# lucadellalib/ts-asr

Hardware: AMD Instinct MI355X
Metric: utterance-frames/sec (conformer-t_scratch training step, T=1000, B=32/GPU) (higher is better)
Workload: dtype bf16; 1 GPU; BASELINE.json configs[1]: conformer-t_scratch 12L d256 (+6L speaker encoder), mel [32,1000,80] + enrollment mel [32,500,80] + tokens [32,120], injection cat, dropout 0.1, lens 1.0; global_batch=32, grad_accumulation_factor=1, parallelism=dp1, hip_graph=True

## Files before the change

### include/tsasr_hip.h

```cpp
#ifndef TSASR_HIP_H
#define TSASR_HIP_H
#include <stddef.h>
#include <stdint.h>

#ifdef __cplusplus
extern "C" {
#endif

#define TSASR_F32 0
#define TSASR_BF16 1

#define TSASR_E_INVALID (-1)
#define TSASR_E_LAUNCH (-2)
#define TSASR_E_WORKSPACE (-3)

const char *tsasr_last_error(void);
int tsasr_version(void);
int tsasr_device_ok(void);

int tsasr_joint_fwd(const void *enc, const void *dec, const float *W, const float *bias, float *logits,
                    int B, int T, int U1, int J, int V, int ldl, int io_dtype, float slope, void *stream);

int tsasr_joint_f32_fwd(const float *enc, const float *dec, const float *W, const float *bias, float *logits, int B, int T, int U1, int J, int V,
                        int ldl, float slope, void *stream);
// ... 82 lines not shown
int tsasr_frontend_out_len(int n);
int tsasr_frontend_c1_fwd(const void *x, const float *w1, const float *b1, const float *w2, const float *b2, void *y1, void *y2,
                          int B, int T, int F, int C, int causal, int io_dtype, void *stream);
size_t tsasr_frontend_c1_bwd_workspace_bytes(int C);
int tsasr_frontend_c1_bwd(const void *x, const void *dy1, const void *dy2, float *dparams, int B, int T, int F, int C, int causal,
                          int io_dtype, void *workspace, size_t workspace_bytes, void *stream);
int tsasr_frontend_im2col(const void *x, void *A, int B, int T, int F, int C, int causal, int io_dtype, void *stream);
int tsasr_frontend_col2im(const void *dA, const void *dR, void *dx, int B, int T, int F, int C, int causal, int io_dtype, void *stream);

int tsasr_frontend_block_supported(int Fo, int C);
int tsasr_frontend_block_fwd(const void *x, const void *y1, const void *y2, const float *w1, const float *b1, const float *w2,
                             const float *b2, const float *g1, const float *be1, const float *g2, const float *be2, void *out,
                             float *stats, int B, int T, int F, int C, int causal, float slope, float eps, float p_inner,
                             unsigned long long seed_inner, float p_outer, unsigned long long seed_outer,
                             const unsigned long long *seed_dev, int io_dtype, void *stream);
size_t tsasr_frontend_block_dparams(int Fo, int C, int with_conv);
size_t tsasr_frontend_block_bwd_workspace_bytes(int Fo, int C, int with_conv);
int tsasr_frontend_block_bwd(const void *x, const void *y1, const void *y2, const void *dout, const float *w1, const float *b1,
                             const float *w2, const float *b2, const float *g1, const float *be1, const float *g2,
                             const float *stats, void *dy1, void *dy2, float *dparams, int B, int T, int F, int C, int causal,
                             float slope, float p_inner, unsigned long long seed_inner, float p_outer,
                             unsigned long long seed_outer, const unsigned long long *seed_dev, int io_dtype, void *workspace,
                             size_t workspace_bytes, void *stream);


size_t tsasr_relpos_attn_lds_bytes(void);
int tsasr_relpos_attn_fwd(const void *qkv, const void *pk, const float *bias_u, const float *bias_v, const int32_t *key_lens,
                          void *out, float *lse, int B, int T, int H, int Dh, float scale, int causal, float pdrop,
                          unsigned long long seed, const unsigned long long *seed_dev, int io_dtype, void *stream);
size_t tsasr_relpos_attn_fwd_workspace_bytes(int B, int T, int H);
int tsasr_relpos_attn_fwd_ws(const void *qkv, const void *pk, const float *bias_u, const float *bias_v, const int32_t *key_lens,
                             void *out, float *lse, int B, int T, int H, int Dh, float scale, int causal, float pdrop,
                             unsigned long long seed, const unsigned long long *seed_dev, int io_dtype, void *workspace,
                             size_t workspace_bytes, void *stream);
size_t tsasr_relpos_attn_bwd_workspace_bytes(int B, int T, int H);
int tsasr_relpos_attn_bwd(const void *qkv, const void *pk, const float *bias_u, const float *bias_v, const int32_t *key_lens,
                          const void *out, const void *dout, const float *lse, void *dqkv, void *dpk, float *d_bias_u,
                          float *d_bias_v, int B, int T, int H, int Dh, float scale, int causal, float pdrop,
                          unsigned long long seed, const unsigned long long *seed_dev, int io_dtype, void *workspace, size_t workspace_bytes,
                          void *stream);
int tsasr_relpos_dpk_defer(int on);
int tsasr_relpos_dpk_pending(void);
size_t tsasr_relpos_dpk_table_bytes(int max_jobs);
int tsasr_relpos_dpk_flush(void *table_host, void *table_dev, size_t table_bytes, void *stream);
void tsasr_relpos_dpk_discard(void);
size_t tsasr_relpos_attn_keepbits_bytes(int B, int T, int H);
void tsasr_relpos_attn_keepbits(void *bits);

int tsasr_accumulate_many(const void *table, int count, void *stream);
size_t tsasr_clip_adamw_workspace_bytes(void);
int tsasr_clip_adamw_step(float *p, void *p_bf16, const float *g, float *m, float *v, const float *hyper, float *norm_out, float *skipped_out,
                          long long n, float beta1, float beta2, float eps, float weight_decay, float max_norm, void *workspace,
                          size_t workspace_bytes, void *stream);

void tsasr_gemm_set_ring(int on);
void tsasr_gemm_set_lab_floor(int floor_mode);
void tsasr_gemm_set_plan(int tile, int splits);
size_t tsasr_gemm_bf16_workspace_bytes(int M, int N, int K, int out_dtype);
int tsasr_gemm_bf16(const void *A, const void *B, void *C, int M, int N, int K, long long lda, long long ldb, long long ldc,
                    int transA, int transB, int out_dtype, int accumulate, void *workspace, size_t workspace_bytes, void *stream);
int tsasr_gemm_f32(const float *A, const float *B, float *C, int M, int N, int K, long long lda, long long ldb, long long ldc, int transA,
                   int transB, int accumulate, void *stream);
int tsasr_gemm_bf16_nt_batched(const void *A, const void *const *btab, void *C, int M, int N, int K, long long lda, long long ldb,
                               long long ldc, long long c_batch, int nbatch, void *stream);
size_t tsasr_gemm_bf16_fused_workspace_bytes(int M, int N);
int tsasr_gemm_bf16_fused_mask_ok(int M, int N, int K);
int tsasr_gemm_bf16_fused(const void *A, const void *B, void *C, int M, int N, int K, long long lda, long long ldb, long long ldc,
                          int transA, int transB, int epi_mode, const float *bias, const void *y, long long ldy, float slope, float p,
                          unsigned long long seed, const unsigned long long *seed_dev, float *dbias, void *mask, void *workspace,
                          size_t workspace_bytes, void *stream);

int tsasr_lstm_cell_fwd(float *gates, float *c, void *h, int B, int U, int H, int t, int io_dtype, void *stream);
int tsasr_lstm_step_fwd(float *gates, float *c, void *h, const void *whh, int B, int U, int H, int t, int io_dtype, void *stream);
int tsasr_lstm_step_bwd(const float *gates, const float *c, const void *dout, void *dgates, const void *whhT, float *dc_io, int B, int U,
                        int H, int t, int io_dtype, void *stream);
int tsasr_lstm_cell_bwd(const float *gates, const float *c, const void *dout, const float *dh_rec, float *dc_io, void *dgates, int B,
                        int U, int H, int t, int io_dtype, void *stream);

size_t tsasr_fbank_workspace_bytes(int B, int T, int n_mels);
int tsasr_fbank_fwd(const float *wav, const float *window, const float *melmat, void *out, int B, int L, int T, int n_mels, int hop,
                    float top_db, float amin, int out_dtype, void *workspace, size_t workspace_bytes, void *stream);
int tsasr_sentence_norm_fwd(const void *x, const int32_t *lens, void *y, int B, int T, int F, float eps, int in_dtype, int out_dtype,
                            void *stream);

size_t tsasr_fbank_frames_workspace_bytes(int n_mels);
int tsasr_fbank_frames(const float *seg, const float *window, const float *melmat, float *out_db, int B, int Lseg, int F, int n_mels, int hop,
                       float amin, void *workspace, size_t workspace_bytes, void *stream);
size_t tsasr_running_norm_state_bytes(int B, int n_mels);
int tsasr_running_norm_fwd(const float *db, const int32_t *n_valid, void *state, void *y, int B, int F, int n_mels, float top_db, double eps,
                           int out_dtype, void *stream);

int tsasr_add_layernorm_fwd(const void *x, const float *bias, const void *res, void *s, void *y, float *mean, float *rstd,
                            const float *gamma, const float *beta, long long M, int D, float alpha, float p, unsigned long long seed,
                            const unsigned long long *seed_dev, const int32_t *valid_lens, int Trows, float eps, int io_dtype,
                            void *stream);
size_t tsasr_add_layernorm_bwd_workspace_bytes(long long M, int D);
int tsasr_add_layernorm_bwd(const void *dy, const void *dout, const void *s, const float *gamma, const float *mean, const float *rstd,
                            void *dres, void *dx, float *dgamma, float *dbeta, float *dbias, long long M, int D, float alpha, float p,
                            unsigned long long seed, const unsigned long long *seed_dev, const int32_t *valid_lens, int Trows,
                            int io_dtype, void *workspace, size_t workspace_bytes, void *stream);
int tsasr_linear_add_layernorm_ok(long long M, int N, int K, long long lda, long long ldw);
int tsasr_linear_add_layernorm_fwd(const void *A, long long lda, const void *W, long long ldw, const float *bias, const void *res, void *s,
                                   void *y, float *mean, float *rstd, const float *gamma, const float *beta, long long M, int N, int K,
                                   float alpha, float p, unsigned long long seed, const unsigned long long *seed_dev,
                                   const int32_t *valid_lens, int Trows, float eps, void *stream);
int tsasr_add_layernorm2_fwd(const void *x, const float *bias, const void *res, void *s, void *y, void *z, float *mean, float *rstd,
// ... 158 lines not shown
```

### ts-asr_amd/_capi.py

```python
import ctypes
import os

_HERE = os.path.dirname(os.path.abspath(__file__))
LIB_PATH = os.environ.get("TSASR_HIP_LIB") or os.path.join(_HERE, "lib", "libtsasr_hip.so")

F32, BF16 = 0, 1


class TsasrHipMissing(RuntimeError):
    pass


class TsasrHipError(RuntimeError):
    pass


_lib = None

c_void_p, c_int, c_float, c_size_t = ctypes.c_void_p, ctypes.c_int, ctypes.c_float, ctypes.c_size_t
c_double = ctypes.c_double
c_ll, c_ull = ctypes.c_longlong, ctypes.c_ulonglong

_PROTOS = {
    "tsasr_last_error": (ctypes.c_char_p, []),
# ... 16 lines not shown
    "tsasr_rnnt_align_workspace_bytes": (c_size_t, [c_int] * 3),
    "tsasr_rnnt_align": (c_int, [c_void_p, c_void_p, c_int, c_void_p, c_void_p, c_void_p, c_int, c_void_p] + [c_int] * 6 + [c_void_p, c_size_t, c_void_p]),
    "tsasr_layernorm_fwd": (c_int, [c_void_p] * 6 + [c_ll, c_int, c_float, c_float, c_int, c_void_p]),
    "tsasr_layernorm_bwd_workspace_bytes": (c_size_t, [c_ll, c_int]),
    "tsasr_layernorm_bwd": (c_int, [c_void_p] * 9 + [c_ll, c_int, c_float, c_int, c_void_p, c_size_t, c_void_p]),
    "tsasr_layernorm_bwd_add": (c_int, [c_void_p] * 10 + [c_ll, c_int, c_float, c_int, c_void_p, c_size_t, c_void_p]),
    "tsasr_seed_advance": (c_int, [c_void_p, c_ull, c_void_p]),
    "tsasr_bias_act_dropout_fwd": (c_int, [c_void_p] * 3 + [c_ll, c_int, c_float, c_float, c_ull, c_void_p, c_int, c_void_p]),
    "tsasr_colpart_workspace_bytes": (c_size_t, [c_ll, c_int]),
    "tsasr_bias_act_dropout_bwd": (c_int, [c_void_p] * 4 + [c_ll, c_int, c_float, c_float, c_ull, c_void_p, c_int, c_void_p, c_size_t, c_void_p]),
    "tsasr_dropout_add_fwd": (c_int, [c_void_p] * 4 + [c_ll, c_int, c_float, c_float, c_ull, c_void_p, c_void_p, c_int, c_int, c_void_p]),
    "tsasr_dropout_add_bwd": (c_int, [c_void_p] * 3 + [c_ll, c_int, c_float, c_float, c_ull, c_void_p, c_void_p, c_int, c_int, c_void_p, c_size_t, c_void_p]),
    "tsasr_dropout_add2_fwd": (c_int, [c_void_p] * 4 + [c_ll, c_int, c_float, c_float, c_ull, c_float, c_ull, c_void_p, c_void_p, c_int, c_int, c_void_p]),
    "tsasr_dropout_add2_bwd": (c_int, [c_void_p] * 4 + [c_ll, c_int, c_float, c_float, c_ull, c_float, c_ull, c_void_p, c_void_p, c_int, c_int, c_void_p, c_size_t, c_void_p]),
    "tsasr_colsum_workspace_bytes": (c_size_t, [c_ll, c_int]),
    "tsasr_colsum": (c_int, [c_void_p, c_void_p, c_ll, c_int, c_int, c_int, c_void_p, c_size_t, c_void_p]),
    "tsasr_convmod_fwd": (c_int, [c_void_p] * 10 + [c_int] * 5 + [c_float, c_float, c_int, c_void_p]),
    "tsasr_convmod_bwd_workspace_bytes": (c_size_t, [c_int] * 4),
    "tsasr_convmod_bwd": (c_int, [c_void_p] * 11 + [c_int] * 5 + [c_float, c_int, c_void_p, c_size_t, c_void_p]),
    "tsasr_frontend_out_len": (c_int, [c_int]),
    "tsasr_frontend_c1_fwd": (c_int, [c_void_p] * 7 + [c_int] * 6 + [c_void_p]),
    "tsasr_frontend_c1_bwd_workspace_bytes": (c_size_t, [c_int]),
    "tsasr_frontend_c1_bwd": (c_int, [c_void_p] * 4 + [c_int] * 6 + [c_void_p, c_size_t, c_void_p]),
    "tsasr_conv3x3s2_fwd": (c_int, [c_void_p] * 7 + [c_int] * 6 + [c_void_p]),
    "tsasr_conv3x3s2_wgrad_workspace_bytes": (c_size_t, [c_int] * 4),
    "tsasr_conv3x3s2_wgrad": (c_int, [c_void_p] * 5 + [c_int] * 6 + [c_void_p, c_size_t, c_void_p]),
    "tsasr_conv3x3s2_wgrad_filters": (c_int, [c_void_p] * 5 + [c_int] * 6 + [c_void_p, c_size_t, c_void_p]),
    "tsasr_conv3x3s2_dgrad_plan_bytes": (c_size_t, [c_int] * 4),
    "tsasr_conv3x3s2_dgrad_plan": (c_int, [c_int] * 4 + [c_void_p, c_size_t]),
    "tsasr_conv3x3s2_dgrad": (c_int, [c_void_p] * 5 + [c_int] * 6 + [c_void_p, c_size_t, c_void_p]),
    "tsasr_frontend_im2col": (c_int, [c_void_p] * 2 + [c_int] * 6 + [c_void_p]),
    "tsasr_frontend_col2im": (c_int, [c_void_p] * 3 + [c_int] * 6 + [c_void_p]),
    "tsasr_frontend_block_supported": (c_int, [c_int, c_int]),
    "tsasr_frontend_block_fwd": (c_int, [c_void_p] * 13 + [c_int] * 5 + [c_float, c_float, c_float, c_ull, c_float, c_ull, c_void_p, c_int, c_void_p]),
    "tsasr_frontend_block_dparams": (c_size_t, [c_int] * 3),
    "tsasr_frontend_block_bwd_workspace_bytes": (c_size_t, [c_int] * 3),
    "tsasr_frontend_block_bwd": (c_int, [c_void_p] * 15 + [c_int] * 5 + [c_float, c_float, c_ull, c_float, c_ull, c_void_p, c_int, c_void_p, c_size_t, c_void_p]),
    "tsasr_relpos_attn_lds_bytes": (c_size_t, []),
    "tsasr_relpos_attn_fwd": (c_int, [c_void_p] * 7 + [c_int] * 4 + [c_float, c_int, c_float, c_ull, c_void_p, c_int, c_void_p]),
    "tsasr_relpos_attn_fwd_workspace_bytes": (c_size_t, [c_int] * 3),
    "tsasr_relpos_attn_fwd_ws": (c_int, [c_void_p] * 7 + [c_int] * 4 + [c_float, c_int, c_float, c_ull, c_void_p, c_int, c_void_p, c_size_t, c_void_p]),
    "tsasr_relpos_attn_bwd_workspace_bytes": (c_size_t, [c_int] * 3),
    "tsasr_relpos_attn_bwd": (c_int, [c_void_p] * 12 + [c_int] * 4 + [c_float, c_int, c_float, c_ull, c_void_p, c_int, c_void_p, c_size_t, c_void_p]),
    "tsasr_relpos_dpk_defer": (c_int, [c_int]),
    "tsasr_relpos_dpk_pending": (c_int, []),
    "tsasr_relpos_dpk_table_bytes": (c_size_t, [c_int]),
    "tsasr_relpos_dpk_flush": (c_int, [c_void_p, c_void_p, c_size_t, c_void_p]),
    "tsasr_relpos_dpk_discard": (None, []),
    "tsasr_relpos_attn_keepbits_bytes": (c_size_t, [c_int] * 3),
    "tsasr_relpos_attn_keepbits": (None, [c_void_p]),
    "tsasr_accumulate_many": (c_int, [c_void_p, c_int, c_void_p]),
    "tsasr_clip_adamw_workspace_bytes": (c_size_t, []),
    "tsasr_clip_adamw_step": (c_int, [c_void_p] * 8 + [c_ll] + [c_float] * 5 + [c_void_p, c_size_t, c_void_p]),
    "tsasr_gemm_set_plan": (None, [c_int, c_int]),
    "tsasr_gemm_set_ring": (None, [c_int]),
    "tsasr_gemm_set_lab_floor": (None, [c_int]),
    "tsasr_gemm_bf16_workspace_bytes": (c_size_t, [c_int] * 4),
    "tsasr_gemm_f32": (c_int, [c_void_p] * 3 + [c_int] * 3 + [c_ll] * 3 + [c_int] * 3 + [c_void_p]),
    "tsasr_gemm_bf16_nt_batched": (c_int, [c_void_p] * 3 + [c_int] * 3 + [c_ll] * 4 + [c_int, c_void_p]),
    "tsasr_gemm_bf16_fused_workspace_bytes": (c_size_t, [c_int] * 2),
    "tsasr_gemm_bf16_fused": (c_int, [c_void_p] * 3 + [c_int] * 3 + [c_ll] * 3 + [c_int] * 3 + [c_void_p, c_void_p, c_ll, c_float, c_float, c_ull, c_void_p, c_void_p, c_void_p, c_void_p, c_size_t, c_void_p]),
    "tsasr_gemm_bf16_fused_mask_ok": (c_int, [c_int] * 3),
    "tsasr_gemm_bf16": (c_int, [c_void_p] * 3 + [c_int] * 3 + [c_ll] * 3 + [c_int] * 4 + [c_void_p, c_size_t, c_void_p]),
    "tsasr_lstm_step_fwd": (c_int, [c_void_p] * 4 + [c_int] * 5 + [c_void_p]),
    "tsasr_lstm_step_bwd": (c_int, [c_void_p] * 6 + [c_int] * 5 + [c_void_p]),
    "tsasr_lstm_cell_fwd": (c_int, [c_void_p] * 3 + [c_int] * 5 + [c_void_p]),
    "tsasr_lstm_cell_bwd": (c_int, [c_void_p] * 6 + [c_int] * 5 + [c_void_p]),
    "tsasr_fbank_workspace_bytes": (c_size_t, [c_int] * 3),
    "tsasr_fbank_fwd": (c_int, [c_void_p] * 4 + [c_int] * 5 + [c_float, c_float, c_int, c_void_p, c_size_t, c_void_p]),
    "tsasr_sentence_norm_fwd": (c_int, [c_void_p] * 3 + [c_int] * 3 + [c_float, c_int, c_int, c_void_p]),
    "tsasr_fbank_frames_workspace_bytes": (c_size_t, [c_int]),
    "tsasr_fbank_frames": (c_int, [c_void_p] * 4 + [c_int] * 5 + [c_float, c_void_p, c_size_t, c_void_p]),
    "tsasr_running_norm_state_bytes": (c_size_t, [c_int] * 2),
    "tsasr_running_norm_fwd": (c_int, [c_void_p] * 4 + [c_int] * 3 + [c_float, c_double, c_int, c_void_p]),
    "tsasr_add_layernorm_fwd": (c_int, [c_void_p] * 9 + [c_ll, c_int, c_float, c_float, c_ull, c_void_p, c_void_p, c_int, c_float, c_int, c_void_p]),
    "tsasr_add_layernorm_bwd_workspace_bytes": (c_size_t, [c_ll, c_int]),
    "tsasr_add_layernorm_bwd": (c_int, [c_void_p] * 11 + [c_ll, c_int, c_float, c_float, c_ull, c_void_p, c_void_p, c_int, c_int, c_void_p, c_size_t, c_void_p]),
    "tsasr_add_layernorm2_fwd": (c_int, [c_void_p] * 14 + [c_ll, c_int, c_float, c_float, c_ull, c_void_p, c_void_p, c_int, c_float, c_float, c_int, c_void_p]),
    "tsasr_add_layernorm2_bwd_workspace_bytes": (c_size_t, [c_ll, c_int]),
    "tsasr_add_layernorm2_bwd": (c_int, [c_void_p] * 18 + [c_ll, c_int, c_float, c_float, c_ull, c_void_p, c_void_p, c_int, c_int, c_void_p, c_size_t, c_void_p]),
    "tsasr_lstm_onehot_gates": (c_int, [c_void_p] * 6 + [c_int] * 6 + [c_void_p]),
    "tsasr_lstm_seq_persistent": (c_int, [c_int, c_int, c_int]),
    "tsasr_lstm_seq_workspace_bytes": (c_size_t, [c_int, c_int, c_int]),
    "tsasr_lstm_seq_fwd": (c_int, [c_void_p] * 4 + [c_int] * 4 + [c_void_p, c_size_t, c_void_p]),
    "tsasr_lstm_seq_bwd": (c_int, [c_void_p] * 5 + [c_int] * 4 + [c_void_p, c_size_t, c_void_p]),
    "tsasr_transpose_many_bf16": (c_int, [c_void_p, c_void_p, c_void_p, c_int, c_int, c_void_p]),
    "tsasr_reduce_defer": (c_int, [c_int]),
    "tsasr_reduce_pending": (c_int, []),
    "tsasr_reduce_discard": (None, []),
    "tsasr_reduce_table_bytes": (c_size_t, [c_int]),
    "tsasr_reduce_flush": (c_int, [c_void_p, c_void_p, c_size_t, c_void_p]),
    "tsasr_reduce_flush_stream": (c_int, [c_void_p, c_void_p, c_size_t, c_void_p]),
    "tsasr_mean_pool_fwd": (c_int, [c_void_p] * 3 + [c_int] * 4 + [c_void_p]),
    "tsasr_mean_pool_bwd": (c_int, [c_void_p] * 3 + [c_int] * 4 + [c_void_p]),
    "tsasr_abs_lengths": (c_int, [c_void_p] * 4 + [c_int, c_int, c_void_p]),
    "tsasr_inject_fwd": (c_int, [c_void_p] * 3 + [c_int] * 5 + [c_void_p]),
    "tsasr_inject_bwd": (c_int, [c_void_p] * 5 + [c_int] * 5 + [c_void_p]),
    "tsasr_greedy_decode": (c_int, [c_void_p] * 12 + [c_int] * 7 + [c_float, c_int, c_int, c_void_p]),
    "tsasr_greedy_decode_stream": (c_int, [c_void_p] * 14 + [c_int] * 7 + [c_float, c_int, c_int, c_void_p]),
    "tsasr_beam_search_workspace_bytes": (c_size_t, [c_int] * 6),
    "tsasr_beam_search": (c_int, [c_void_p] * 11 + [c_size_t] + [c_void_p] * 4 + [c_int] * 11 + [c_double, c_double, c_float, c_int, c_int, c_void_p]),
    "tsasr_beam_search_stream": (c_int, [c_void_p] * 11 + [c_size_t] + [c_void_p] * 5 + [c_int] * 12 + [c_double, c_double, c_float, c_int, c_int, c_void_p]),
    "tsasr_beam_search_timed_workspace_bytes": (c_size_t, [c_int] * 6),
    "tsasr_beam_search_timed": (c_int, [c_void_p] * 11 + [c_size_t] + [c_void_p] * 4 + [c_int] * 11 + [c_double, c_double, c_float, c_int, c_int, c_void_p, c_void_p]),
    "tsasr_beam_search_stream_timed": (c_int, [c_void_p] * 11 + [c_size_t] + [c_void_p] * 5 + [c_int] * 12 + [c_double, c_double, c_float, c_int, c_int, c_void_p, c_void_p]),
    "tsasr_beam_search_lm_workspace_bytes": (c_size_t, [c_int] * 9),
# ... 117 lines not shown
```

### ts-asr_amd/csrc/optim.hip

```cpp
#include <float.h>

#include "common.h"

#define OPT_PARTS 1024

__global__ __launch_bounds__(256) void sumsq_partials_kernel(const float *__restrict__ g, float *__restrict__ part, long long n) {
    __shared__ float red[4];
    const long long per = (((n + OPT_PARTS - 1) / OPT_PARTS) + 3) & ~3ll;
    const long long lo = min(n, (long long)blockIdx.x * per), hi = min(n, lo + per);
    const long long hi4 = lo + ((hi - lo) & ~3ll);
    float s0 = 0.f, s1 = 0.f, s2 = 0.f, s3 = 0.f;
    long long i = lo + threadIdx.x * 4;
    for (; i + 3 * 1024 + 4 <= hi4; i += 4 * 1024) {
        const float4 a = *reinterpret_cast<const float4 *>(g + i), b = *reinterpret_cast<const float4 *>(g + i + 1024);
        const float4 c = *reinterpret_cast<const float4 *>(g + i + 2048), d = *reinterpret_cast<const float4 *>(g + i + 3072);
        s0 += a.x * a.x + a.y * a.y + a.z * a.z + a.w * a.w;
        s1 += b.x * b.x + b.y * b.y + b.z * b.z + b.w * b.w;
        s2 += c.x * c.x + c.y * c.y + c.z * c.z + c.w * c.w;
        s3 += d.x * d.x + d.y * d.y + d.z * d.z + d.w * d.w;
    }
    for (; i + 4 <= hi4; i += 1024) {
        const float4 a = *reinterpret_cast<const float4 *>(g + i);
        s0 += a.x * a.x + a.y * a.y + a.z * a.z + a.w * a.w;
    }
// ... 38 lines not shown
        for (int i = threadIdx.x; i < OPT_PARTS; i += 256) s2 += part[OPT_PARTS + i];
        s2 = wave_sum(s2);
        __syncthreads();
        if ((threadIdx.x & 63) == 0) red[threadIdx.x >> 6] = s2;
        __syncthreads();
        norm = sqrtf(red[0] + red[1] + red[2] + red[3]) * 0x1p64f;
    }
    if (blockIdx.x == 0 && threadIdx.x == 0 && norm_out) *norm_out = norm;
    const bool finite = fabsf(norm) <= FLT_MAX;
    if (!finite && skipped_out) {
        if (blockIdx.x == 0 && threadIdx.x == 0) *skipped_out += 1.f;
        return;
    }
    float clip = 1.f;
    if (max_norm > 0.f) {
        const float c = max_norm / (norm + 1e-6f);
        clip = (c != c) ? c : fminf(1.f, c);
    }
    const float lr = hyper[0], bc1 = hyper[1], bc2s = sqrtf(hyper[2]);
    const float step = lr / bc1, decay = 1.f - lr * wd;
    for (long long i = ((long long)blockIdx.x * 256 + threadIdx.x) * 4; i < n; i += (long long)gridDim.x * 256 * 4) {
        if (i + 4 <= n) {
            float4 pp = *reinterpret_cast<float4 *>(p + i), mm = *reinterpret_cast<float4 *>(m + i), vv = *reinterpret_cast<float4 *>(v + i);
            const float4 gg = *reinterpret_cast<const float4 *>(g + i);
            float *P = &pp.x, *M = &mm.x, *V = &vv.x;
            const float *G = &gg.x;
#pragma unroll
            for (int k = 0; k < 4; ++k) {
                const float gk = G[k] * clip;
                M[k] = beta1 * M[k] + (1.f - beta1) * gk;
                V[k] = beta2 * V[k] + (1.f - beta2) * gk * gk;
                P[k] = P[k] * decay - step * M[k] / (sqrtf(V[k]) / bc2s + eps);
            }
            *reinterpret_cast<float4 *>(p + i) = pp;
            if (p16) {
                bf16x4 h4;
                h4[0] = (bf16_t)pp.x; h4[1] = (bf16_t)pp.y; h4[2] = (bf16_t)pp.z; h4[3] = (bf16_t)pp.w;
                *reinterpret_cast<bf16x4 *>(p16 + i) = h4;
            }
            *reinterpret_cast<float4 *>(m + i) = mm;
            *reinterpret_cast<float4 *>(v + i) = vv;
        } else {
            for (long long k = i; k < n; ++k) {
                const float gk = g[k] * clip;
                m[k] = beta1 * m[k] + (1.f - beta1) * gk;
                v[k] = beta2 * v[k] + (1.f - beta2) * gk * gk;
                p[k] = p[k] * decay - step * m[k] / (sqrtf(v[k]) / bc2s + eps);
                if (p16) p16[k] = (bf16_t)p[k];
            }
        }
    }
}

#define ACC_SPLIT 16
__global__ __launch_bounds__(256) void accumulate_many_kernel(const float *const *__restrict__ src, float *const *__restrict__ dst,
                                                              const int *__restrict__ n) {
    const float *s = src[blockIdx.x];
    float *d = dst[blockIdx.x];
    const int len = n[blockIdx.x];
    for (int i = blockIdx.y * 256 + threadIdx.x; i < len; i += 256 * ACC_SPLIT) d[i] += s[i];
}

__global__ __launch_bounds__(256) void transpose_many_bf16_kernel(const unsigned short *__restrict__ src_base, unsigned short *__restrict__ dst_base,
                                                                  const int *__restrict__ jobs, int njobs) {
    __shared__ unsigned short tile[64][66];
    int lo = 0, hi = njobs - 1;
    const int bid = blockIdx.x;
    while (lo < hi) {
        const int mid = (lo + hi + 1) >> 1;
        if (jobs[mid * 5 + 4] <= bid) lo = mid; else hi = mid - 1;
    }
    const int *jb = jobs + lo * 5;
    const int rows = jb[2], cols = jb[3], lt = bid - jb[4], tcn = (cols + 63) >> 6;
    const int r0 = (lt / tcn) * 64, c0 = (lt % tcn) * 64;
    const unsigned short *src = src_base + jb[0];
    unsigned short *dst = dst_base + jb[1];
    if (r0 + 64 <= rows && c0 + 64 <= cols && (cols & 7) == 0 && (rows & 7) == 0 && ((jb[0] | jb[1]) & 7) == 0) {
        uint4 v[2];
#pragma unroll
        for (int i = 0; i < 2; ++i) {
            const int q = threadIdx.x + 256 * i, row = q >> 3, c8 = (q & 7) * 8;
            v[i] = *reinterpret_cast<const uint4 *>(src + (size_t)(r0 + row) * cols + c0 + c8);
        }
#pragma unroll
        for (int i = 0; i < 2; ++i) {
            const int q = threadIdx.x + 256 * i, row = q >> 3, c8 = (q & 7) * 8;
            unsigned *t32 = reinterpret_cast<unsigned *>(&tile[row][c8]);
            t32[0] = v[i].x; t32[1] = v[i].y; t32[2] = v[i].z; t32[3] = v[i].w;
        }
        __syncthreads();
#pragma unroll
        for (int i = 0; i < 2; ++i) {
            const int q = threadIdx.x + 256 * i, c = q >> 3, r8 = (q & 7) * 8;
            unsigned short e[8];
#pragma unroll
            for (int j = 0; j < 8; ++j) e[j] = tile[r8 + j][c];
            uint4 o;
            o.x = e[0] | ((unsigned)e[1] << 16); o.y = e[2] | ((unsigned)e[3] << 16);
            o.z = e[4] | ((unsigned)e[5] << 16); o.w = e[6] | ((unsigned)e[7] << 16);
            *reinterpret_cast<uint4 *>(dst + (size_t)(c0 + c) * rows + r0 + r8) = o;
        }
        return;
    }
    const int cx = threadIdx.x & 63, ry = threadIdx.x >> 6;
#pragma unroll
    for (int i = 0; i < 16; ++i) {
        const int r = r0 + ry + 4 * i, c = c0 + cx;
        tile[ry + 4 * i][cx] = (r < rows && c < cols) ? src[(size_t)r * cols + c] : (unsigned short)0;
    }
    __syncthreads();
#pragma unroll
    for (int i = 0; i < 16; ++i) {
        const int c = c0 + ry + 4 * i, r = r0 + cx;
        if (c < cols && r < rows) dst[(size_t)c * rows + r] = tile[cx][ry + 4 * i];
    }
}

extern "C" {

int tsasr_accumulate_many(const void *table, int count, void *stream) {
    TSASR_CHECK_ARG(table && count > 0, "tsasr_accumulate_many: bad arguments");
    const float *const *src = (const float *const *)table;
    float *const *dst = (float *const *)((const char *)table + (size_t)count * sizeof(void *));
    const int *n = (const int *)((const char *)table + (size_t)2 * count * sizeof(void *));
    accumulate_many_kernel<<<dim3(count, ACC_SPLIT), 256, 0, (hipStream_t)stream>>>(src, dst, n);
    TSASR_CHECK_LAUNCH("tsasr_accumulate_many");
    return 0;
}

size_t tsasr_clip_adamw_workspace_bytes(void) { return 2 * OPT_PARTS * sizeof(float); }

int tsasr_clip_adamw_step(float *p, void *p_bf16, const float *g, float *m, float *v, const float *hyper, float *norm_out, float *skipped_out, long long n,
                          float beta1, float beta2, float eps, float weight_decay, float max_norm, void *workspace,
                          size_t workspace_bytes, void *stream) {
    TSASR_CHECK_ARG(p && g && m && v && hyper && workspace, "tsasr_clip_adamw_step: null pointer");
    TSASR_CHECK_ARG(n > 0 && workspace_bytes >= tsasr_clip_adamw_workspace_bytes(), "tsasr_clip_adamw_step: bad size / workspace");
    TSASR_CHECK_ARG((((uintptr_t)p | (uintptr_t)g | (uintptr_t)m | (uintptr_t)v) & 15) == 0, "tsasr_clip_adamw_step: buffers must be 16-byte aligned");
    hipStream_t st = (hipStream_t)stream;
    float *part = (float *)workspace;
    sumsq_partials_kernel<<<OPT_PARTS, 256, 0, st>>>(g, part, n);
    long long blocks = ((n + 3) / 4 + 255) / 256;
    if (blocks > 2048) blocks = 2048;
    clip_adamw_kernel<<<(unsigned)blocks, 256, 0, st>>>(p, (bf16_t *)p_bf16, g, m, v, part, hyper, norm_out, skipped_out, n, beta1, beta2, eps, weight_decay, max_norm);
    TSASR_CHECK_LAUNCH("tsasr_clip_adamw_step");
    return 0;
}

int tsasr_transpose_many_bf16(const void *src_base, void *dst_base, const void *jobs, int njobs, int ntiles, void *stream) {
    TSASR_CHECK_ARG(src_base && dst_base && jobs && njobs > 0 && ntiles > 0, "tsasr_transpose_many_bf16: bad arguments");
    transpose_many_bf16_kernel<<<ntiles, 256, 0, (hipStream_t)stream>>>((const unsigned short *)src_base, (unsigned short *)dst_base, (const int *)jobs, njobs);
    TSASR_CHECK_LAUNCH("tsasr_transpose_many_bf16");
    return 0;
}

}
```

### ts-asr_amd/dp.py

```python
import ctypes
import os

import torch
import torch.distributed as dist


def is_initialized():
    return dist.is_available() and dist.is_initialized()


def world_size():
    return dist.get_world_size() if is_initialized() else 1


def ddp_init_group(run_opts):
    if not run_opts.get("distributed_launch", False) or is_initialized():
        return
    if "RANK" not in os.environ or "LOCAL_RANK" not in os.environ:
        raise ValueError("To use DDP backend, start your script with:\n\tpython -m torch.distributed.run "
                         "--nproc-per-node=N train.py hparams.yaml --distributed_launch --distributed_backend=nccl")
    backend = run_opts.get("distributed_backend", "nccl")
    if backend not in ("nccl", "gloo", "mpi"):
        raise ValueError(backend + " communication protocol doesn't exist.")
    if backend == "nccl":
# ... 23 lines not shown
        dist.broadcast_object_list(box, src=0)
        uid = torch.frombuffer(bytearray(box[0]), dtype=torch.uint8).clone()
    torch.cuda.set_device(torch.device(device))
    C.check(lib.tsasr_allreduce_init(C.ptr(uid), world, rank), "tsasr_allreduce_init")
    _DIRECT["ranks"] = world
    return world


def direct_capture_probe(device, world, rank, group=None):
    import sys
    from . import _capi as C

    def agree(flag_value):
        if is_initialized() and world > 1:
            flag = torch.tensor([int(flag_value)], dtype=torch.int32, device=device if dist.get_backend(group) == "nccl" else "cpu")
            dist.all_reduce(flag, op=dist.ReduceOp.MIN, group=group)
            return int(flag.item())
        return int(flag_value)

    ok, g, buf = 1, None, None
    try:
        buf = torch.full((4096,), float(rank + 1), dtype=torch.float32, device=device)
        comm = torch.cuda.Stream(device=device)
        torch.cuda.synchronize()
        g = torch.cuda.CUDAGraph()
        with torch.cuda.graph(g, capture_error_mode="thread_local"):
            cur = torch.cuda.current_stream()
            comm.wait_stream(cur)
            C.check(C.lib().tsasr_allreduce_bucket(C.ptr(buf), buf.numel(), C.F32, 1, ctypes.c_void_p(comm.cuda_stream)), "tsasr_allreduce_bucket")
            cur.wait_stream(comm)
    except Exception as e:
        print(f"[ts-asr_amd] rank {rank}: capturing an RCCL all-reduce failed ({type(e).__name__}: {e})", file=sys.stderr, flush=True)
        ok = 0
    if not agree(ok):
        return False
    try:
        g.replay()
        torch.cuda.synchronize()
        n = _DIRECT["ranks"] or world
        ok = int(bool(torch.allclose(buf, torch.full_like(buf, (n + 1) / 2.0), rtol=1e-6)))
        if not ok:
            print(f"[ts-asr_amd] rank {rank}: captured all-reduce replayed a wrong average ({float(buf[0])})", file=sys.stderr, flush=True)
    except Exception as e:
        print(f"[ts-asr_amd] rank {rank}: replaying a captured RCCL all-reduce failed ({type(e).__name__}: {e})", file=sys.stderr, flush=True)
        ok = 0
    return bool(agree(ok))


_PAD = 64


def _pad8(n):
    return (int(n) + _PAD - 1) // _PAD * _PAD


class GradArena:
    def __init__(self, modules, world_size=1, bucket_bytes=None, group=None):
        if bucket_bytes is None:
            bucket_bytes = int(float(os.environ.get("TSASR_BUCKET_MB", "32")) * (1 << 20))
        seen, params = set(), []
        for p in modules.parameters():
            if p.requires_grad and id(p) not in seen:
                seen.add(id(p))
                params.append(p)
        if not params:
            raise ValueError("no trainable parameters")
        self.params_ordered = params
        self.params_initial = list(params)
        self.world_size, self.group, self.bucket_bytes = world_size, group, bucket_bytes
        self.comm_dtype = os.environ.get("TSASR_ALLREDUCE_DTYPE", "fp32")
        self.direct = bool(world_size > 1 and direct_rccl_init(world_size, dist.get_rank() if is_initialized() else 0, params[0].device))
        self.comm_stream = None
        self.device = params[0].device
        self.numel = sum(_pad8(p.numel()) for p in params)
        self.grads = torch.zeros(self.numel, dtype=torch.float32, device=self.device)
        self.flat_params = torch.zeros(self.numel, dtype=torch.float32, device=self.device)
        self.flat_params16 = torch.empty(self.numel, dtype=torch.bfloat16, device=self.device) if self.device.type == "cuda" else None
        self.in_backward = False
        self.sync_enabled = True
        self._sync_this_step = False
        self._order_seen, self._order_final = [], False
        self._contrib, self._contrib_step = {}, {}
        self._handles, self.sent_log, self._next_send = [], [], 0
        self.probe = None
        self.aux_streams, self._main_stream = [], None
        self.companions = []
        self._deferred, self._keepalive, self._defer_ring = [], None, None
        self.collect_wgrads = self.device.type == "cuda"
        self._wgrad_hold, self._wgrad_held = [], False
        self._reorder_pending = False
        self._layout(params, first=True)
        self._hooks = [p.register_post_accumulate_grad_hook(self._on_grad) for p in params]
        if self.device.type == "cuda":
            from . import ops
            self._defer_ring = ops.TableRing(max(1024, 2 * len(params)) * 20, self.device)
            ops.reduce_defer_prepare(self.device)

    def _layout(self, params, first=False):
        new_off, off = {}, 0
        for p in params:
            new_off[id(p)] = off
            off += _pad8(p.numel())
        if first:
            for p in params:
                o, n = new_off[id(p)], p.numel()
                self.flat_params[o:o + n].copy_(p.data.reshape(-1).float())
        else:
            for buf in [self.flat_params] + self.companions:
                old = buf.clone()
                buf.zero_()
                for p in params:
                    o, n, oo = new_off[id(p)], p.numel(), self.offset[id(p)]
                    buf[o:o + n].copy_(old[oo:oo + n])
        self.offset = new_off
        for p in params:
            o, n = new_off[id(p)], p.numel()
            p.data = self.flat_params[o:o + n].view(p.shape)
            p.grad = self.grads[o:o + n].view(p.shape)
        self.params_ordered = list(params)
        self.refresh_shadow()
        self.buckets, start, pend = [], 0, []
        limit = max(1, self.bucket_bytes // 4)
        for p in params:
            pend.append(id(p))
            end = self.offset[id(p)] + p.numel()
            if end - start >= limit:
                self.buckets.append({"lo": start, "hi": end, "ids": set(pend), "left": len(pend)})
                start, pend = end, []
        if pend:
            self.buckets.append({"lo": start, "hi": self.numel, "ids": set(pend), "left": len(pend)})
        self.bucket_of = {i: b for b in self.buckets for i in b["ids"]}

    def refresh_shadow(self):
        if self.flat_params16 is None:
            return
        self.flat_params16.copy_(self.flat_params)
        jobs, t_off, tiles = [], 0, 0
        mats = [p for p in self.params_ordered if (p.dim() == 2 or (p.dim() == 3 and p.shape[2] == 1)) and min(p.shape[:2]) >= 16 and p.numel() >= 4096]
        total_t = sum(_pad8(p.numel()) for p in mats)
        if getattr(self, "flat_params16_t", None) is None or self.flat_params16_t.numel() != total_t:
            self.flat_params16_t = torch.empty(max(total_t, 1), dtype=torch.bfloat16, device=self.device)
        for p in self.params_ordered:
            o, n = self.offset[id(p)], p.numel()
            p._bf16 = self.flat_params16[o:o + n].view(p.shape)
            p._bf16_ver = p._version
            p._bf16_t = None
        for p in mats:
            r, c = p.shape[0], p.shape[1]
            jobs.append((self.offset[id(p)], t_off, r, c, tiles))
            p._bf16_t = self.flat_params16_t[t_off:t_off + r * c].view(c, r)
            t_off += _pad8(r * c)
            tiles += ((r + 63) // 64) * ((c + 63) // 64)
        self._tr_njobs, self._tr_tiles = len(jobs), tiles
        self._tr_jobs = torch.tensor(jobs, dtype=torch.int32).reshape(-1).to(self.device) if jobs else None
        self.refresh_transposed()

    def sync_shadow(self):
        if self.flat_params16 is None:
            return
        self.flat_params16.copy_(self.flat_params)
        for p in self.params_ordered:
            p._bf16_ver = p._version
        self.refresh_transposed()

    def refresh_transposed(self):
        if getattr(self, "_tr_jobs", None) is None:
            return
        from . import _capi as C
        C.check(C.lib().tsasr_transpose_many_bf16(C.ptr(self.flat_params16), C.ptr(self.flat_params16_t), C.ptr(self._tr_jobs),
                                                  self._tr_njobs, self._tr_tiles, C.stream_ptr()), "tsasr_transpose_many_bf16")

    def accepts(self, p):
        return self.in_backward and id(p) in self.offset and p.grad is not None

    def mark_ready(self, p):
        self._on_grad(p)

    def defer_add(self, p, g):
        if self._sync_this_step or not self.accepts(p) or g.dtype != torch.float32 or not g.is_cuda or g.numel() != p.numel():
            return False
        self._deferred.append((g.contiguous(), p))
        return True

    def _flush_deferred(self):
        if not self._deferred:
            return
        import numpy as np
        from . import _capi as C
        n = len(self._deferred)
        from . import ops
        if self._defer_ring is None:
            self._defer_ring = ops.TableRing(max(1024, 2 * n) * 20, self.device)
        k, host, dev, captured = self._defer_ring.acquire()
        if host.numel() < n * 20:
            raise RuntimeError("deferred-gradient table too small")
        tab = np.empty(n * 20, np.uint8)
        tab[:n * 8].view(np.uint64)[:] = [g.data_ptr() for g, _ in self._deferred]
        tab[n * 8:n * 16].view(np.uint64)[:] = [p.grad.data_ptr() for _, p in self._deferred]
        tab[n * 16:].view(np.int32)[:] = [g.numel() for g, _ in self._deferred]
        host[:n * 20].copy_(torch.from_numpy(tab))
        if not captured:
            dev[:n * 20].copy_(host[:n * 20], non_blocking=True)
        C.check(C.lib().tsasr_accumulate_many(C.ptr(dev), n, C.stream_ptr()), "tsasr_accumulate_many")
        self._defer_ring.launched(k, n * 20)
        self._keepalive = self._deferred
        self._deferred = []

# ... 202 lines not shown
```

### ts-asr_amd/optim.py

```python
import functools

import torch

from . import _capi as C
from . import prof


_HYPER_SLOTS = 64

class FusedClipAdamW:

    def __init__(self, arena, lr=1e-3, betas=(0.9, 0.999), eps=1e-8, weight_decay=1e-2, max_grad_norm=0.0, skip_nonfinite=False):
        self.arena = arena
        self.skip_nonfinite = bool(skip_nonfinite)
        self.param_groups = [{"lr": lr, "betas": tuple(betas), "eps": eps, "weight_decay": weight_decay,
                              "params": arena.params_ordered}]
        self.max_grad_norm = float(max_grad_norm or 0.0)
        self.exp_avg = torch.zeros_like(arena.grads)
        self.exp_avg_sq = torch.zeros_like(arena.grads)
        arena.companions += [self.exp_avg, self.exp_avg_sq]
        self.t = 0
        self._norm_buf = torch.zeros(2, device=arena.device)
        self.last_grad_norm = self._norm_buf[0]
        self._hyper_host = self._hyper_dev = self._ws = None

    def prepare(self):
        g = self.param_groups[0]
        self.t += 1
        b1, b2 = g["betas"]
        cuda = self.arena.device.type == "cuda"
        if self._hyper_host is None:
            self._hyper_host = torch.empty(_HYPER_SLOTS, 3, dtype=torch.float32).pin_memory() if cuda else torch.empty(_HYPER_SLOTS, 3)
            self._hyper_events = [None] * _HYPER_SLOTS
            self._hyper_dev = torch.empty(3, dtype=torch.float32, device=self.arena.device)
            self._ws = torch.empty(max(256, C.lib().tsasr_clip_adamw_workspace_bytes()), dtype=torch.uint8, device=self.arena.device)
        k = self.t % _HYPER_SLOTS
        if cuda and self._hyper_events[k] is not None:
            self._hyper_events[k].synchronize()
        row = self._hyper_host[k]
        row[0], row[1], row[2] = g["lr"], 1.0 - b1 ** self.t, 1.0 - b2 ** self.t
        self._hyper_dev.copy_(row, non_blocking=True)
        if cuda:
            ev = self._hyper_events[k] or torch.cuda.Event()
            ev.record()
            self._hyper_events[k] = ev

    def launch(self):
        g = self.param_groups[0]
        a = self.arena
        b1, b2 = g["betas"]
        C.require_gpu(a.flat_params)
        with prof.region("clip_adamw"):
            C.check(C.lib().tsasr_clip_adamw_step(C.ptr(a.flat_params), C.ptr(a.flat_params16), C.ptr(a.grads), C.ptr(self.exp_avg),
                                                  C.ptr(self.exp_avg_sq), C.ptr(self._hyper_dev), C.ptr(self._norm_buf[0:1]),
                                                  C.ptr(self._norm_buf[1:2]) if self.skip_nonfinite else None, a.numel,
                                                  float(b1), float(b2), float(g["eps"]), float(g["weight_decay"]), self.max_grad_norm,
                                                  C.ptr(self._ws), self._ws.numel(), C.stream_ptr()), "tsasr_clip_adamw_step")
            a.refresh_transposed()

    def step(self):
        self.prepare()
        self.launch()

    def take_skipped_steps(self):
        n = int(self._norm_buf[1].item())
        if n:
            self._norm_buf[1].zero_()
        return n

    def zero_grad(self, set_to_none=False):
        self.arena.zero_()

    def state_dict(self):
        return {"t": self.t, "exp_avg": self.exp_avg, "exp_avg_sq": self.exp_avg_sq, "param_groups": [
            {k: v for k, v in self.param_groups[0].items() if k != "params"}]}


def _clip_adamw(p, g, m, v, norm_out, lr, b1, b2, eps, wd, t, max_norm, p16=None, skipped_out=None):
    C.require_gpu(p, g, m, v)
    hyper = torch.tensor([lr, 1.0 - b1 ** t, 1.0 - b2 ** t], dtype=torch.float32).to(p.device)
    ws = torch.empty(max(256, C.lib().tsasr_clip_adamw_workspace_bytes()), dtype=torch.uint8, device=p.device)
    C.check(C.lib().tsasr_clip_adamw_step(C.ptr(p), C.ptr(p16), C.ptr(g), C.ptr(m), C.ptr(v), C.ptr(hyper), C.ptr(norm_out), C.ptr(skipped_out), p.numel(),
                                          float(b1), float(b2), float(eps), float(wd), float(max_norm), C.ptr(ws), ws.numel(),
                                          C.stream_ptr()), "tsasr_clip_adamw_step")


class _WrappedTorchOptimizer:

    def __init__(self, opt, arena, max_grad_norm):
        self.opt, self.arena, self.max_grad_norm = opt, arena, float(max_grad_norm or 0.0)
        self.param_groups = opt.param_groups
        self.last_grad_norm = torch.zeros((), device=arena.device)

    def prepare(self):
        pass

    def launch(self):
        norm = self.arena.grad_norm()
        self.last_grad_norm.copy_(norm)
        if self.max_grad_norm > 0:
            self.arena.grads.mul_(torch.clamp(self.max_grad_norm / (norm + 1e-6), max=1.0))
        self.opt.step()
        self.arena.sync_shadow()

    def step(self):
        self.launch()

    def zero_grad(self, set_to_none=False):
        self.arena.zero_()

# ... 8 lines not shown
```

Measured before the change: 3.306 million frames/s.

## Fuse bf16 transposed-weight refresh into the clipped AdamW update kernel

```diff
diff --git a/include/tsasr_hip.h b/include/tsasr_hip.h
--- a/include/tsasr_hip.h
+++ b/include/tsasr_hip.h
@@ -158,6 +158,9 @@
 int tsasr_clip_adamw_step(float *p, void *p_bf16, const float *g, float *m, float *v, const float *hyper, float *norm_out, float *skipped_out,
                           long long n, float beta1, float beta2, float eps, float weight_decay, float max_norm, void *workspace,
                           size_t workspace_bytes, void *stream);
+int tsasr_clip_adamw_step_t(float *p, void *p_bf16, void *p_bf16_t, const float *g, float *m, float *v, const float *hyper, float *norm_out,
+                            float *skipped_out, long long n, const void *jobs, int njobs, int nitems, float beta1, float beta2, float eps,
+                            float weight_decay, float max_norm, void *workspace, size_t workspace_bytes, void *stream);
 
 void tsasr_gemm_set_ring(int on);
 void tsasr_gemm_set_lab_floor(int floor_mode);
diff --git a/ts-asr_amd/_capi.py b/ts-asr_amd/_capi.py
--- a/ts-asr_amd/_capi.py
+++ b/ts-asr_amd/_capi.py
@@ -92,6 +92,7 @@
     "tsasr_accumulate_many": (c_int, [c_void_p, c_int, c_void_p]),
     "tsasr_clip_adamw_workspace_bytes": (c_size_t, []),
     "tsasr_clip_adamw_step": (c_int, [c_void_p] * 8 + [c_ll] + [c_float] * 5 + [c_void_p, c_size_t, c_void_p]),
+    "tsasr_clip_adamw_step_t": (c_int, [c_void_p] * 9 + [c_ll, c_void_p, c_int, c_int] + [c_float] * 5 + [c_void_p, c_size_t, c_void_p]),
     "tsasr_gemm_set_plan": (None, [c_int, c_int]),
     "tsasr_gemm_set_ring": (None, [c_int]),
     "tsasr_gemm_set_lab_floor": (None, [c_int]),
diff --git a/ts-asr_amd/csrc/optim.hip b/ts-asr_amd/csrc/optim.hip
--- a/ts-asr_amd/csrc/optim.hip
+++ b/ts-asr_amd/csrc/optim.hip
@@ -114,6 +114,189 @@
     }
 }
 
+
+struct AdamStep {
+    float clip, step, decay, bc2s, beta1, beta2, eps;
+};
+
+__device__ __forceinline__ void adamw_elem(float &p, float &m, float &v, const float g, const AdamStep &a) {
+#pragma clang fp contract(off)
+    const float gk = g * a.clip;
+    m = fmaf(a.beta1, m, (1.f - a.beta1) * gk);
+    v = fmaf((1.f - a.beta2) * gk, gk, a.beta2 * v);
+    p = fmaf(p, a.decay, -(a.step * m / (sqrtf(v) / a.bc2s + a.eps)));
+}
+
+__device__ __forceinline__ bool adam_step_head(const float *__restrict__ part, const float *__restrict__ hyper, float *__restrict__ norm_out,
+                                               float *__restrict__ skipped_out, float *red, float beta1, float beta2, float eps, float wd,
+                                               float max_norm, AdamStep &a) {
+    float s = 0.f;
+    for (int i = threadIdx.x; i < OPT_PARTS; i += 256) s += part[i];
+    s = wave_sum(s);
+    if ((threadIdx.x & 63) == 0) red[threadIdx.x >> 6] = s;
+    __syncthreads();
+    const float sumsq = red[0] + red[1] + red[2] + red[3];
+    float norm = sqrtf(sumsq);
+    if (sumsq == INFINITY) {
+        float s2 = 0.f;
+        for (int i = threadIdx.x; i < OPT_PARTS; i += 256) s2 += part[OPT_PARTS + i];
+        s2 = wave_sum(s2);
+        __syncthreads();
+        if ((threadIdx.x & 63) == 0) red[threadIdx.x >> 6] = s2;
+        __syncthreads();
+        norm = sqrtf(red[0] + red[1] + red[2] + red[3]) * 0x1p64f;
+    }
+    if (blockIdx.x == 0 && threadIdx.x == 0 && norm_out) *norm_out = norm;
+    const bool finite = fabsf(norm) <= FLT_MAX;
+    if (!finite && skipped_out) {
+        if (blockIdx.x == 0 && threadIdx.x == 0) *skipped_out += 1.f;
+        return false;
+    }
+    a.clip = 1.f;
+    if (max_norm > 0.f) {
+        const float c = max_norm / (norm + 1e-6f);
+        a.clip = (c != c) ? c : fminf(1.f, c);
+    }
+    const float lr = hyper[0], bc1 = hyper[1];
+    a.bc2s = sqrtf(hyper[2]);
+    a.step = lr / bc1;
+    a.decay = fmaf(-lr, wd, 1.f);
+    a.beta1 = beta1, a.beta2 = beta2, a.eps = eps;
+    return true;
+}
+
+__device__ __forceinline__ void adamw_group4(float *__restrict__ p, bf16_t *__restrict__ p16, const float *__restrict__ g, float *__restrict__ m,
+                                             float *__restrict__ v, long long i, const AdamStep &a) {
+    float4 pp = *reinterpret_cast<float4 *>(p + i), mm = *reinterpret_cast<float4 *>(m + i), vv = *reinterpret_cast<float4 *>(v + i);
+    const float4 gg = *reinterpret_cast<const float4 *>(g + i);
+    float *P = &pp.x, *M = &mm.x, *V = &vv.x;
+    const float *G = &gg.x;
+#pragma unroll
+    for (int k = 0; k < 4; ++k) adamw_elem(P[k], M[k], V[k], G[k], a);
+    *reinterpret_cast<float4 *>(p + i) = pp;
+    if (p16) {
+        bf16x4 h4;
+        h4[0] = (bf16_t)pp.x; h4[1] = (bf16_t)pp.y; h4[2] = (bf16_t)pp.z; h4[3] = (bf16_t)pp.w;
+        *reinterpret_cast<bf16x4 *>(p16 + i) = h4;
+    }
+    *reinterpret_cast<float4 *>(m + i) = mm;
+    *reinterpret_cast<float4 *>(v + i) = vv;
+}
+
+__device__ __forceinline__ void adamw_scalar(float *__restrict__ p, bf16_t *__restrict__ p16, const float *__restrict__ g, float *__restrict__ m,
+                                             float *__restrict__ v, long long lo, long long hi, const AdamStep &a) {
+    for (long long k = lo; k < hi; ++k) {
+        adamw_elem(p[k], m[k], v[k], g[k], a);
+        if (p16) p16[k] = (bf16_t)p[k];
+    }
+}
+
+#define OPT_FLAT_ITEM 1024
+__global__ __launch_bounds__(256) void clip_adamw_tiles_kernel(float *__restrict__ p, bf16_t *__restrict__ p16, unsigned short *__restrict__ p16t,
+                                                               const float *__restrict__ g, float *__restrict__ m, float *__restrict__ v,
+                                                               const float *__restrict__ part, const float *__restrict__ hyper,
+                                                               float *__restrict__ norm_out, float *__restrict__ skipped_out,
+                                                               const int *__restrict__ jobs, int njobs, float beta1, float beta2, float eps,
+                                                               float wd, float max_norm) {
+    __shared__ float red[4];
+    __shared__ unsigned short tile[64][66];
+    AdamStep a;
+    if (!adam_step_head(part, hyper, norm_out, skipped_out, red, beta1, beta2, eps, wd, max_norm, a)) return;
+    const int tid = threadIdx.x, lane = tid & 63;
+    const int w = blockIdx.x;
+    int lo = 0, cnt = njobs;
+    while (cnt > 1) {
+        const int stp = (cnt + 63) >> 6;
+        const bool le = lane * stp < cnt && jobs[(lo + lane * stp) * 5 + 4] <= w;
+        const int seg = __popcll(__ballot(le)) - 1;
+        lo += seg * stp;
+        cnt = min(stp, cnt - seg * stp);
+    }
+    lo = __builtin_amdgcn_readfirstlane(lo);
+    const int *jb = jobs + lo * 5;
+    const long long off = jb[0], toff = jb[1];
+    const int rows = jb[2], cols = jb[3], it = w - jb[4];
+    if (cols == 0) {
+        const long long hi = off + rows, i = (off & ~3ll) + ((long long)it * 256 + tid) * 4;
+        if (i >= off && i + 4 <= hi) adamw_group4(p, p16, g, m, v, i, a);
+        else adamw_scalar(p, p16, g, m, v, max(i, off), min(i + 4, hi), a);
+        return;
+    }
+    const int tcn = (cols + 63) >> 6, r0 = (it / tcn) * 64, c0 = (it % tcn) * 64;
+    unsigned short *dst = p16t + toff;
+    if (r0 + 64 <= rows && c0 + 64 <= cols && (cols & 7) == 0 && (rows & 7) == 0 && ((off | toff) & 7) == 0) {
+        const int c4 = (tid & 15) * 4, rr = tid >> 4;
+        float4 P[4], G[4], M[4], V[4];
+#pragma unroll
+        for (int i = 0; i < 4; ++i) {
+            const long long e = off + (long long)(r0 + rr + 16 * i) * cols + c0 + c4;
+            P[i] = *reinterpret_cast<const float4 *>(p + e); G[i] = *reinterpret_cast<const float4 *>(g + e);
+            M[i] = *reinterpret_cast<const float4 *>(m + e); V[i] = *reinterpret_cast<const float4 *>(v + e);
+        }
+#pragma unroll
+        for (int i = 0; i < 4; ++i) {
+            const long long e = off + (long long)(r0 + rr + 16 * i) * cols + c0 + c4;
+            float *Pk = &P[i].x, *Mk = &M[i].x, *Vk = &V[i].x;
+            const float *Gk = &G[i].x;
+#pragma unroll
+            for (int k = 0; k < 4; ++k) adamw_elem(Pk[k], Mk[k], Vk[k], Gk[k], a);
+            *reinterpret_cast<float4 *>(p + e) = P[i];
+            bf16x4 h4;
+            h4[0] = (bf16_t)P[i].x; h4[1] = (bf16_t)P[i].y; h4[2] = (bf16_t)P[i].z; h4[3] = (bf16_t)P[i].w;
+            *reinterpret_cast<bf16x4 *>(p16 + e) = h4;
+            *reinterpret_cast<float4 *>(m + e) = M[i];
+            *reinterpret_cast<float4 *>(v + e) = V[i];
+            const uint2 hb = __builtin_bit_cast(uint2, h4);
+            unsigned *t32 = reinterpret_cast<unsigned *>(&tile[rr + 16 * i][c4]);
+            t32[0] = hb.x; t32[1] = hb.y;
+        }
+        __syncthreads();
+#pragma unroll
+        for (int i = 0; i < 2; ++i) {
+            const int q = tid + 256 * i, c = q >> 3, r8 = (q & 7) * 8;
+            unsigned short e[8];
+#pragma unroll
+            for (int j = 0; j < 8; ++j) e[j] = tile[r8 + j][c];
+            uint4 o;
+            o.x = e[0] | ((unsigned)e[1] << 16); o.y = e[2] | ((unsigned)e[3] << 16);
+            o.z = e[4] | ((unsigned)e[5] << 16); o.w = e[6] | ((unsigned)e[7] << 16);
+            *reinterpret_cast<uint4 *>(dst + (size_t)(c0 + c) * rows + r0 + r8) = o;
+        }
+    } else {
+        const int cx = tid & 63, ry = tid >> 6;
+        const int cg = c0 + cx;
+        for (int i0 = 0; i0 < 16; i0 += 4) {
+            float P[4], G[4], M[4], V[4];
+#pragma unroll
+            for (int i = 0; i < 4; ++i) {
+                const int r = r0 + ry + 4 * (i0 + i);
+                const bool in = r < rows && cg < cols;
+                const long long e = off + (long long)r * cols + cg;
+                P[i] = in ? p[e] : 0.f; G[i] = in ? g[e] : 0.f; M[i] = in ? m[e] : 0.f; V[i] = in ? v[e] : 0.f;
+            }
+#pragma unroll
+            for (int i = 0; i < 4; ++i) {
+                const int r = r0 + ry + 4 * (i0 + i);
+                unsigned short hb = 0;
+                if (r < rows && cg < cols) {
+                    const long long e = off + (long long)r * cols + cg;
+                    adamw_elem(P[i], M[i], V[i], G[i], a);
+                    const bf16_t h = (bf16_t)P[i];
+                    p[e] = P[i]; m[e] = M[i]; v[e] = V[i]; p16[e] = h;
+                    hb = __builtin_bit_cast(unsigned short, h);
+                }
+                tile[ry + 4 * (i0 + i)][cx] = hb;
+            }
+        }
+        __syncthreads();
+#pragma unroll
+        for (int i = 0; i < 16; ++i) {
+            const int c = c0 + ry + 4 * i, r = r0 + cx;
+            if (c < cols && r < rows) dst[(size_t)c * rows + r] = tile[cx][ry + 4 * i];
+        }
+    }
+}
+
 #define ACC_SPLIT 16
 __global__ __launch_bounds__(256) void accumulate_many_kernel(const float *const *__restrict__ src, float *const *__restrict__ dst,
                                                               const int *__restrict__ n) {
@@ -208,6 +391,23 @@
     return 0;
 }
 
+int tsasr_clip_adamw_step_t(float *p, void *p_bf16, void *p_bf16_t, const float *g, float *m, float *v, const float *hyper, float *norm_out,
+                            float *skipped_out, long long n, const void *jobs, int njobs, int nitems, float beta1, float beta2, float eps,
+                            float weight_decay, float max_norm, void *workspace, size_t workspace_bytes, void *stream) {
+    TSASR_CHECK_ARG(p && p_bf16 && p_bf16_t && g && m && v && hyper && workspace && jobs, "tsasr_clip_adamw_step_t: null pointer");
+    TSASR_CHECK_ARG(n > 0 && n < (1ll << 31) && njobs > 0 && nitems >= njobs && workspace_bytes >= tsasr_clip_adamw_workspace_bytes(),
+                    "tsasr_clip_adamw_step_t: bad size / job table / workspace");
+    TSASR_CHECK_ARG((((uintptr_t)p | (uintptr_t)g | (uintptr_t)m | (uintptr_t)v | (uintptr_t)p_bf16 | (uintptr_t)p_bf16_t) & 15) == 0,
+                    "tsasr_clip_adamw_step_t: buffers must be 16-byte aligned");
+    hipStream_t st = (hipStream_t)stream;
+    float *part = (float *)workspace;
+    sumsq_partials_kernel<<<OPT_PARTS, 256, 0, st>>>(g, part, n);
+    clip_adamw_tiles_kernel<<<nitems, 256, 0, st>>>(p, (bf16_t *)p_bf16, (unsigned short *)p_bf16_t, g, m, v, part, hyper, norm_out, skipped_out,
+                                                    (const int *)jobs, njobs, beta1, beta2, eps, weight_decay, max_norm);
+    TSASR_CHECK_LAUNCH("tsasr_clip_adamw_step_t");
+    return 0;
+}
+
 int tsasr_transpose_many_bf16(const void *src_base, void *dst_base, const void *jobs, int njobs, int ntiles, void *stream) {
     TSASR_CHECK_ARG(src_base && dst_base && jobs && njobs > 0 && ntiles > 0, "tsasr_transpose_many_bf16: bad arguments");
     transpose_many_bf16_kernel<<<ntiles, 256, 0, (hipStream_t)stream>>>((const unsigned short *)src_base, (unsigned short *)dst_base, (const int *)jobs, njobs);
diff --git a/ts-asr_amd/dp.py b/ts-asr_amd/dp.py
--- a/ts-asr_amd/dp.py
+++ b/ts-asr_amd/dp.py
@@ -99,6 +99,31 @@
 
 def _pad8(n):
     return (int(n) + _PAD - 1) // _PAD * _PAD
+
+
+_OPT_FLAT_ITEM = 1024
+
+
+def optimizer_jobs(mats, numel):
+    jobs, items, pos = [], 0, 0
+
+    def flat(lo, hi):
+        nonlocal items
+        if hi > lo:
+            jobs.append((lo, 0, hi - lo, 0, items))
+            items += (hi - (lo & ~3) + _OPT_FLAT_ITEM - 1) // _OPT_FLAT_ITEM
+
+    for off, t_off, r, c in mats:
+        if off < pos or r < 1 or c < 1:
+            raise ValueError(f"optimizer_jobs: matrix [{r}, {c}] at {off} overlaps its predecessor (ends at {pos}) or is empty")
+        flat(pos, off)
+        jobs.append((off, t_off, r, c, items))
+        items += ((r + 63) // 64) * ((c + 63) // 64)
+        pos = off + r * c
+    if pos > numel:
+        raise ValueError(f"optimizer_jobs: the last matrix ends at {pos}, behind the arena's {numel} elements")
+    flat(pos, numel)
+    return jobs, items
 
 
 class GradArena:
@@ -200,6 +225,11 @@
             tiles += ((r + 63) // 64) * ((c + 63) // 64)
         self._tr_njobs, self._tr_tiles = len(jobs), tiles
         self._tr_jobs = torch.tensor(jobs, dtype=torch.int32).reshape(-1).to(self.device) if jobs else None
+        self._opt_jobs = None
+        if jobs and self.numel < 2 ** 31:
+            rows, self._opt_items = optimizer_jobs([j[:4] for j in jobs], self.numel)
+            self._opt_njobs = len(rows)
+            self._opt_jobs = torch.tensor(rows, dtype=torch.int32).reshape(-1).to(self.device)
         self.refresh_transposed()
 
     def sync_shadow(self):
diff --git a/ts-asr_amd/optim.py b/ts-asr_amd/optim.py
--- a/ts-asr_amd/optim.py
+++ b/ts-asr_amd/optim.py
@@ -1,4 +1,5 @@
 import functools
+import os
 
 import torch
 
@@ -13,6 +14,7 @@
     def __init__(self, arena, lr=1e-3, betas=(0.9, 0.999), eps=1e-8, weight_decay=1e-2, max_grad_norm=0.0, skip_nonfinite=False):
         self.arena = arena
         self.skip_nonfinite = bool(skip_nonfinite)
+        self.fused_transpose = os.environ.get("TSASR_ADAMW_TRANSPOSE", "1") != "0"
         self.param_groups = [{"lr": lr, "betas": tuple(betas), "eps": eps, "weight_decay": weight_decay,
                               "params": arena.params_ordered}]
         self.max_grad_norm = float(max_grad_norm or 0.0)
@@ -50,12 +52,18 @@
         a = self.arena
         b1, b2 = g["betas"]
         C.require_gpu(a.flat_params)
+        skipped = C.ptr(self._norm_buf[1:2]) if self.skip_nonfinite else None
+        adam = (float(b1), float(b2), float(g["eps"]), float(g["weight_decay"]), self.max_grad_norm, C.ptr(self._ws), self._ws.numel(), C.stream_ptr())
         with prof.region("clip_adamw"):
+            if self.fused_transpose and a.flat_params16 is not None and getattr(a, "_opt_jobs", None) is not None:
+                C.check(C.lib().tsasr_clip_adamw_step_t(C.ptr(a.flat_params), C.ptr(a.flat_params16), C.ptr(a.flat_params16_t), C.ptr(a.grads),
+                                                        C.ptr(self.exp_avg), C.ptr(self.exp_avg_sq), C.ptr(self._hyper_dev), C.ptr(self._norm_buf[0:1]),
+                                                        skipped, a.numel, C.ptr(a._opt_jobs), a._opt_njobs, a._opt_items, *adam),
+                        "tsasr_clip_adamw_step_t")
+                return
             C.check(C.lib().tsasr_clip_adamw_step(C.ptr(a.flat_params), C.ptr(a.flat_params16), C.ptr(a.grads), C.ptr(self.exp_avg),
-                                                  C.ptr(self.exp_avg_sq), C.ptr(self._hyper_dev), C.ptr(self._norm_buf[0:1]),
-                                                  C.ptr(self._norm_buf[1:2]) if self.skip_nonfinite else None, a.numel,
-                                                  float(b1), float(b2), float(g["eps"]), float(g["weight_decay"]), self.max_grad_norm,
-                                                  C.ptr(self._ws), self._ws.numel(), C.stream_ptr()), "tsasr_clip_adamw_step")
+                                                  C.ptr(self.exp_avg_sq), C.ptr(self._hyper_dev), C.ptr(self._norm_buf[0:1]), skipped, a.numel, *adam),
+                    "tsasr_clip_adamw_step")
             a.refresh_transposed()
 
     def step(self):
```

Measured after the change: 3.314 million frames/s, median of 4. Within noise of the previous version (+0.2%).
